# marthinwurer/gcmiipy

Hardware: AMD Instinct MI355X
Metric: cell-updates/s (C-grid Matsuno step) (higher is better)
Workload: dtype f64; 1 GPU; 2-D shallow water + theta + viscosity + van-Leer tracer, 4096x2048 fp64 (BASELINE configs[2]); variant=fused, decomposition=1 latitude band(s)

## Files before the change

gcmiipy_amd/_lib.py:

```python
import ctypes as C
import os

_HERE = os.path.dirname(os.path.abspath(__file__))
LIB_PATH = os.environ.get("GCMCORE_LIB", os.path.join(_HERE, "lib", "libgcmcore.so"))

ABI_VERSION = 1

SW2D, SW2D_TEMP, PE2D, PE25D = 1, 2, 3, 4
P, U, V, T, Q = 0, 1, 2, 3, 4
TRACER_NONE, TRACER_UPWIND, TRACER_VANLEER = 0, 1, 2
VARIANT_AUTO, VARIANT_STAGED, VARIANT_FUSED = 0, 1, 2
F64, F32 = 0, 1
MAX_TRACERS = 16
TRACER_STATS_WORDS = 6
CLIM_WORDS3, CLIM_WORDS2 = 10, 2
PLEV_MAX, PLEV_WORDS, PLEV_PLAN_WORDS = 64, 13, 6
PLEV_MAP_WORDS, PLEV_MAP_WORDS2, PLEV_MAP_PLAN_WORDS = 13, 2, 5
SPEC_WORDS = 6
SPEC_PLAN_WORDS = 6
HDIFF_U, HDIFF_V, HDIFF_T, HDIFF_Q = 1, 2, 4, 8
HDIFF_PLAN_WORDS = 7
SW2D_PLAN_WORDS = 9
PHASE_HELD_SUAREZ, PHASE_MOIST, PHASE_CLIMATE, PHASE_TRACER_FORCING = range(4)
PHASE_PLAN_WORDS = 5
# ... 89 lines not shown
    "gcm_build_info": (C.c_char_p, []),
    "gcm_exner_table": (C.c_int, [_dp]),
    "gcm_filter_plan": (C.c_int, [C.c_int, C.POINTER(C.c_uint), C.c_int]),
    "gcm_create": (C.c_int, [C.POINTER(Config), C.POINTER(_H)]),
    "gcm_destroy": (C.c_int, [_H]),
    "gcm_last_error": (C.c_char_p, [_H]),
    "gcm_set_state": (C.c_int, [_H] + [C.c_void_p] * 5),
    "gcm_get_state": (C.c_int, [_H] + [C.c_void_p] * 5),
    "gcm_members": (C.c_int, [_H]),
    "gcm_set_member": (C.c_int, [_H, C.c_int] + [C.c_void_p] * 5),
    "gcm_get_member": (C.c_int, [_H, C.c_int] + [C.c_void_p] * 5),
    "gcm_diag_members": (C.c_int, [_H, C.c_int, _dp, C.c_int]),
    "gcm_step": (C.c_int, [_H, C.c_int, C.c_double]),
    "gcm_sw2d_plan": (C.c_int, [_H, C.c_int, C.POINTER(C.c_int), C.c_int]),
    "gcm_sw2d_fused_depth": (C.c_int, [_H]),
    "gcm_pe25d_phase_geometry": (C.c_int, [C.c_int] * 7 + [C.POINTER(C.c_int), C.c_int]),
    "gcm_pe25d_phase_plan": (C.c_int, [_H, C.c_int, C.c_int, C.c_int, C.POINTER(C.c_int), C.c_int]),
    "gcm_pe25d_stage_geometry": (C.c_int, [C.c_int] * 5 + [C.POINTER(C.c_uint), C.c_int, C.POINTER(C.c_int), C.c_int]),
    "gcm_pe25d_stage_plan": (C.c_int, [_H, C.POINTER(C.c_int), C.c_int]),
    "gcm_half_step": (C.c_int, [_H, C.c_int, C.c_double]),
    "gcm_end_step": (C.c_int, [_H, C.c_double]),
    "gcm_end_step_diffuse": (C.c_int, [_H, C.c_double]),
    "gcm_end_step_begin": (C.c_int, [_H, C.c_double]),
    "gcm_end_step_finish": (C.c_int, [_H, C.c_double]),
    "gcm_get_star": (C.c_int, [_H] + [C.c_void_p] * 5),
    "gcm_set_star": (C.c_int, [_H] + [C.c_void_p] * 5),
    "gcm_diag": (C.c_int, [_H, C.c_int, _dp]),
    "gcm_energy": (C.c_int, [_H, _dp, C.c_int, _dp]),
    "gcm_stats": (C.c_int, [_H, _dp, C.c_int, _dp]),
    "gcm_flux_limiter": (C.c_int, [C.c_int, C.c_int, C.c_void_p, C.c_void_p, C.c_double, C.c_double, C.c_void_p]),
# ... 168 lines not shown
```

gcmiipy_amd/core.py:

```python
import collections
import ctypes as C

import numpy as np

from . import _lib
from ._lib import lib


class GcmError(RuntimeError):
    pass


def _check(rc, h=None):
    if rc == _lib.OK:
        return
    msg = lib.gcm_last_error(h).decode() if (h or rc) else ""
    if rc == _lib.ERR_ARG:
        raise ValueError(msg or "gcmcore: bad argument")
    raise GcmError("gcmcore error %d: %s" % (rc, msg))


def _count(n, h):
    if n < 0:
        _check(n, h)
# ... 855 lines not shown
    def band_tracer_rows(self):
        return _count(lib.gcm_band_tracer_rows(self._h), self._h)

    @property
    def tracer_count(self):
        return _count(lib.gcm_tracer_count(self._h), self._h)

    def step(self, nsteps, dt):
        _check(lib.gcm_step(self._h, int(nsteps), float(dt)), self._h)

    def sw2d_fused_depth(self):
        d = lib.gcm_sw2d_fused_depth(self._h)
        _check(min(d, 0), self._h)
        return d

    def sw2d_plan(self, nsteps):
        out = (C.c_int * _lib.SW2D_PLAN_WORDS)()
        _check(lib.gcm_sw2d_plan(self._h, int(nsteps), out, _lib.SW2D_PLAN_WORDS), self._h)
        return dict(variant={_lib.VARIANT_FUSED: "fused", _lib.VARIANT_STAGED: "staged"}[out[0]],
                    rows_per_band=out[1], cols=out[2], strip=out[3], strip2=out[4], two_step_launches=out[5],
                    single_step_launches=out[6], preload=bool(out[7]), stream=bool(out[8]))

    def phase_plan(self, phase, rows=None, accumulate=True):
        out = (C.c_int * _lib.PHASE_PLAN_WORDS)()
        _check(lib.gcm_pe25d_phase_plan(self._h, phase_id(phase), -1 if rows is None else int(rows), int(bool(accumulate)),
                                        out, _lib.PHASE_PLAN_WORDS), self._h)
        return _phase_dict(phase_id(phase), out)

    def stage_plan(self):
        out = (C.c_int * _lib.STAGE_PLAN_WORDS)()
# ... 509 lines not shown
```

gcmiipy_amd/csrc/gcm_handle.h:

```cpp
#pragma once
#include "../../include/gcmcore.h"

#include <hip/hip_runtime.h>

#include <algorithm>
#include <cstdio>
#include <string>
#include <vector>

#include "pe25d_kernels.h"
#include "sw2d_kernels.h"

struct GcmBandExchange {
    gcm_exchange xch{};
    bool set = false, primed = false;
    bool inflight = false;
    bool overlap = false;
    hipEvent_t ev_pack = nullptr, ev_comm = nullptr;
    bool join_pending = false;
    bool on_comm = false;
};

struct GcmTiming {
    bool on = false;
// ... 28 lines not shown
    int since_exchange = 0;
    bool ghosts_current = false;
    bool star_valid = false;
    bool launch_refused = false;
    hipStream_t comm = nullptr;
    double *snap[GCM_NFIELDS] = {};
    int snap_since_exchange = 0;
    int variant = GCM_VARIANT_FUSED;
    int rows_per_band = 32;
    int M = 1;
    long mstride = 0;
    bool f32 = false;
    int esz = 8;
    int cols = 1;
    int depth_pin = 0;
    double *staging = nullptr;
    int staging_members = 0;

    double *diag_dev = nullptr;
    static constexpr int kDiagBlocks = 512;

    GcmTiming time;
    gcm::Pe25d *pe = nullptr;
    GcmBandExchange band;
    GcmPhases phases;
};

#define HIPCHK(h, call)                                                                    \
    do {                                                                                   \
        hipError_t e_ = (call);                                                            \
// ... 63 lines not shown
```

gcmiipy_amd/csrc/gcmcore.hip:

```cpp
#include <cmath>
#include <cstdlib>
#include <cstring>

#include "gcm_handle.h"

using namespace gcm;

std::string &gcm_create_error() {
    thread_local std::string e;
    return e;
}

static int alloc_field(gcm_handle *h, double **p) {
    static const long skew_unit = getenv("GCM_ALLOC_SKEW") ? atol(getenv("GCM_ALLOC_SKEW")) : 256;
    const size_t n = all_members_elems(h);
    const size_t skew = (size_t)(skew_unit > 0 ? skew_unit : 0) * (h->allocs.size() % 16) / h->esz;
    void *d = nullptr;
    HIPCHK(h, hipMalloc(&d, (n + skew) * h->esz));
    HIPCHK(h, hipMemsetAsync(d, 0, (n + skew) * h->esz, h->stream));
    h->allocs.push_back(d);
    *p = at(h, (double *)d, (long)(skew + (size_t)h->G * h->W));
    return GCM_OK;
}

// ... 119 lines not shown
                if ((rc = alloc_field(h, &h->cur[f]))) return bail(rc, "");
                if ((rc = alloc_field(h, &h->nxt[f]))) return bail(rc, "");
                if (f != GCM_Q && (rc = alloc_field(h, &h->star[f]))) return bail(rc, "");
            }
            if (temp) {
                if ((rc = alloc_field(h, &h->geo))) return bail(rc, "");
                if ((rc = alloc_field(h, &h->irho))) return bail(rc, "");
                if ((rc = alloc_field(h, &h->sst))) return bail(rc, "");
            }
            if (h->has[GCM_Q] && (rc = alloc_field(h, &h->qtmp))) return bail(rc, "");
            if (temp && !upload_exner_table(h)) return bail(GCM_ERR_HIP, "gcm_create: exner table upload failed");
            const int tr = h->has[GCM_Q] ? cfg->tracer : 0;
            if (h->f32) h->cols = sw2d_fused_cols<float>(h->W, h->H, temp, tr, h->wrap, h->M);
            if (const char *e = getenv("GCM_SW2D_DEPTH"))
                if (temp && !h->f32 && (e[0] == '1' || e[0] == '3') && !e[1]) h->depth_pin = e[0] - '0';
            h->rows_per_band = h->f32 ? sw2d_fused_rows_per_band<float>(h->W, h->H, temp, tr, h->wrap, h->M, h->cols)
                                      : sw2d_fused_rows_per_band<double>(h->W, h->H, temp, tr, h->wrap, h->M, 1, h->depth_pin);
            break;
        }
        case GCM_PE2D: {
            if (!(cfg->dx > 0)) return bail(GCM_ERR_ARG, "gcm_create: dx must be > 0");
            if (cfg->nranks != 1)
                return bail(GCM_ERR_UNSUPPORTED, "gcm_create: GCM_PE2D has no latitude-band mode");
            h->variant = GCM_VARIANT_STAGED;
            for (int f = 0; f < GCM_NFIELDS; ++f) {
                h->has[f] = true;
                if ((rc = alloc_field(h, &h->cur[f]))) return bail(rc, "");
                if ((rc = alloc_field(h, &h->nxt[f]))) return bail(rc, "");
                if ((rc = alloc_field(h, &h->star[f]))) return bail(rc, "");
            }
            if (!upload_exner_table(h)) return bail(GCM_ERR_HIP, "gcm_create: exner table upload failed");
            break;
// ... 139 lines not shown

static void run_derive(const gcm_handle *h, const Sw2dArgs &a, hipStream_t s) {
    if (h->f32) launch_sw2d_derive(narrow_args(a), s);
    else launch_sw2d_derive(a, s);
}
static void run_stage(const gcm_handle *h, const Sw2dArgs &a, bool temp, hipStream_t s) {
    if (h->f32) launch_sw2d_stage(narrow_args(a), temp, s);
    else launch_sw2d_stage(a, temp, s);
}
static void run_tracer_axis(const gcm_handle *h, const Sw2dArgs &a, int axis, bool limit, const double *q_in,
                            double *q_out, hipStream_t s) {
    if (h->f32) launch_tracer_axis(narrow_args(a), axis, limit, (const float *)q_in, (float *)q_out, s);
    else launch_tracer_axis(a, axis, limit, q_in, q_out, s);
}
static bool run_fused(const gcm_handle *h, const Sw2dArgs &a, bool temp, int tracer, hipStream_t s) {
    return h->f32 ? launch_sw2d_fused(narrow_args(a), temp, tracer, s, h->cols) : launch_sw2d_fused(a, temp, tracer, s, 1, h->depth_pin);
}
static bool run_fused2(const gcm_handle *h, const Sw2dArgs &a, hipStream_t s) {
    return h->f32 ? launch_sw2d_fused2(narrow_args(a), s) : launch_sw2d_fused2(a, s);
}

int launch_status(gcm_handle *h) {
    const hipError_t e = hipGetLastError();
    if (h->launch_refused) {
        h->launch_refused = false;
        return fail(h, GCM_ERR_HIP, std::string("sw2d fused kernel: launch refused") +
                                        (e != hipSuccess ? std::string(": ") + hipGetErrorString(e) : std::string()));
    }
    HIPCHK(h, e);
    return GCM_OK;
}
// ... 143 lines not shown
    out[5] = pairs;
    out[6] = nsteps - 2 * pairs;
    out[7] = f.preload;
    out[8] = f.stream;
    return GCM_OK;
}

int gcm_sw2d_fused_depth(gcm_handle *h) {
    if (!h || h->pe) return GCM_ERR_ARG;
    if (h->variant != GCM_VARIANT_FUSED) return 0;
    const int e = step_extra_rows(h);
    return sw2d_fused_form(h->cfg.model == GCM_SW2D_TEMP, h->has[GCM_Q] ? h->cfg.tracer : 0, h->rows_per_band, h->W,
                           h->H + 2 * e, h->M, h->esz, h->depth_pin).depth;
}

int gcm_step_interior(gcm_handle *h, double dt, void *stream) {
    if (!h) return GCM_ERR_ARG;
    if (h->pe) return pe25d_step_part(h->pe, 0, dt, (hipStream_t)stream, &h->err);
    if (h->wrap) return fail(h, GCM_ERR_STATE, "step_interior: handle is not a latitude band");
    if (h->G != kGhost) return fail(h, GCM_ERR_STATE, "step_interior: halo_steps > 1 steps through gcm_step");
    step_rows(h, dt, kGhost, h->H - kGhost, (hipStream_t)stream);
    return launch_status(h);
}

int gcm_step_boundary(gcm_handle *h, double dt, void *stream) {
    if (!h) return GCM_ERR_ARG;
    if (h->pe) return pe25d_step_part(h->pe, 1, dt, (hipStream_t)stream, &h->err);
    if (h->wrap) return fail(h, GCM_ERR_STATE, "step_boundary: handle is not a latitude band");
    hipStream_t s = (hipStream_t)stream;
    if (h->H <= 2 * kGhost) {
// ... 210 lines not shown
```

gcmiipy_amd/csrc/sw2d_impl.h:

```cpp
#pragma once
#include <hip/hip_runtime.h>

#include <cstdlib>
#include <type_traits>

#include "gcm_math.h"
#include "sw2d_kernels.h"

namespace gcm {

__device__ __forceinline__ long row_off(int j, int H, int W, bool wrap) {
    if (wrap) {
        j %= H;
        if (j < 0) j += H;
    }
    return (long)j * W;
}

template <typename T>
__device__ __forceinline__ Sw2dArgsT<T> member_args(const Sw2dArgsT<T> &a0, int m) {
    Sw2dArgsT<T> a = a0;
    const long o = (long)m * a0.mstride;
    auto mv = [o](auto *p) { return p ? p + o : p; };
    a.bu = mv(a.bu); a.bv = mv(a.bv); a.bp = mv(a.bp); a.bt = mv(a.bt); a.bq = mv(a.bq);
// ... 192 lines not shown
};

constexpr unsigned kNoStore = 0x80000000u;
__device__ __forceinline__ void store_row_lanes(double *row, int W, unsigned lane_off, double x) {
    typedef unsigned int u32x2 __attribute__((ext_vector_type(2)));
    const __amdgpu_buffer_rsrc_t rs = __builtin_amdgcn_make_buffer_rsrc(row, 0, W * 8, 0x00020000);
    __builtin_amdgcn_raw_buffer_store_b64(__builtin_bit_cast(u32x2, x), rs, (int)lane_off, 0, 0);
}

__device__ __forceinline__ double own_copy(double x) {
    double y;
    asm volatile("v_mov_b64 %0, %1" : "=v"(y) : "v"(x) : "memory");
    return y;
}

template <typename T, bool TEMP, int TRACER, bool WRAPJ, bool STREAM = false, int CPL = 1>
struct FusedCtx {
    using Real = std::conditional_t<CPL == 2, f32x2, T>;
    using V = Real;
    const Sw2dArgsT<T> &a;
    const double *tab;
    int ci, col, ja, jb;
    bool store_lane;
    V f0_prev;

    __device__ __forceinline__ Raw<V> load(int j) const {
        const long o = row_off(j, a.H, a.W, WRAPJ) + ci;
        Raw<V> r;
        if constexpr (CPL == 2) {
            auto ld = [o](const T *p) {
                const f32x2 *q = (const f32x2 *)(p + o);
                return STREAM ? __builtin_nontemporal_load(q) : *q;
            };
            r.u = ld(a.bu);
            r.v = ld(a.bv);
            r.p = ld(a.bp);
            r.t = TEMP ? ld(a.bt) : V(0.0f);
            r.q = TRACER ? ld(a.bq) : V(0.0f);
        } else if (STREAM) {
            r.u = __builtin_nontemporal_load(&a.bu[o]);
            r.v = __builtin_nontemporal_load(&a.bv[o]);
            r.p = __builtin_nontemporal_load(&a.bp[o]);
            r.t = TEMP ? __builtin_nontemporal_load(&a.bt[o]) : T(0.0);
            r.q = TRACER ? __builtin_nontemporal_load(&a.bq[o]) : T(0.0);
        } else {
            r.u = a.bu[o];
            r.v = a.bv[o];
            r.p = a.bp[o];
            r.t = TEMP ? a.bt[o] : T(0.0);
            r.q = TRACER ? a.bq[o] : T(0.0);
        }
        return r;
    }

// ... 77 lines not shown
};

template <int N, int PRE, class Ctx, typename T = typename Ctx::Real>
__device__ __forceinline__ void preloaded_iters(Ctx &c, const Raw<T> (&pre)[PRE + 4], Row<T> &A, Row<T> &B, Row<T> &C,
                                                Row<T> &X, Row<T> &Y, Row<T> &Z, Raw<T> &nxt, T &qmm, T &qm, T &q0,
                                                T &qp) {
    if constexpr (N < PRE + 2) {
        const int r = c.ja - 1 + N;
        if (r > c.jb) return;
        c.template iter<false>(r, A, B, C, X, Y, Z, nxt, qmm, qm, q0, qp);
        if constexpr (N < PRE) nxt = pre[N + 4];
        preloaded_iters<N + 1, PRE>(c, pre, B, C, A, Y, Z, X, nxt, qmm, qm, q0, qp);
    }
}

template <typename T, bool TEMP, int TRACER, bool WRAPJ, int PRE = 0, bool STREAM = false, int CPL = 1, int DEPTH = 1>
__global__ __launch_bounds__(64, DEPTH == 3 ? 2 : (CPL == 2 && TRACER != 0) ? 3 : 1) void sw2d_fused_kernel(Sw2dArgsT<T> a0) {
    using Ctx = FusedCtx<T, TEMP, TRACER, WRAPJ, STREAM, CPL>;
    using V = typename Ctx::Real;
    constexpr int kCols = sw2d_fused_strip_cols(CPL);
    const int W = a0.W;
    const int lane = threadIdx.x;
    const int strips = (W + kCols - 1) / kCols;
    const int per_xcd = gridDim.x / 8;
    int tile = (blockIdx.x % 8) * per_xcd + blockIdx.x / 8;
    int member = 0;
    if (a0.members > 1) {
        const int per_member = strips * ((a0.j1 - a0.j0 + a0.rows_per_band - 1) / a0.rows_per_band);
        member = tile / per_member;
        if (member >= a0.members) return;
        tile -= member * per_member;
    }
    const int band = tile / strips;
    const int i0 = (tile - band * strips) * kCols;
    const Sw2dArgsT<T> a = member_args(a0, member);
    __shared__ double tab[kExnerTabDoubles];
    if (TEMP) {
        for (int k = 0; k < kExnerTabDoubles / 64; ++k) tab[lane + 64 * k] = a.exner_tab[lane + 64 * k];
        __syncthreads();
    }
    Ctx c{a, tab};
    c.ja = a.j0 + band * a.rows_per_band;
    c.jb = min(c.ja + a.rows_per_band, a.j1);
    if (c.ja >= c.jb) return;
    c.col = i0 - 2 * CPL + CPL * lane;
    c.ci = c.col % W;
    if (c.ci < 0) c.ci += W;
    c.store_lane = lane >= 2 && lane < 62 && c.col < W;
    c.f0_prev = V(0.0);
    const int ja = c.ja, jb = c.jb;

    Row<V> A, B, C, X, Y, Z;
    if constexpr (PRE > 0) {
        Raw<V> pre[PRE + 4];
#pragma unroll
        for (int n = 0; n < PRE + 4; ++n) pre[n] = c.load(min(ja - 2 + n, jb + 1));
        make_row<TEMP>(A, pre[0].u, pre[0].v, pre[0].p, pre[0].t, tab);
        make_row<TEMP>(B, pre[1].u, pre[1].v, pre[1].p, pre[1].t, tab);
        make_row<TEMP>(C, pre[2].u, pre[2].v, pre[2].p, pre[2].t, tab);
        V qmm = V(0.0), qm = pre[0].q, q0 = pre[1].q, qp = pre[2].q;
        Raw<V> nxt = pre[3];
        X = Y = Z = A;
        preloaded_iters<0, PRE>(c, pre, A, B, C, X, Y, Z, nxt, qmm, qm, q0, qp);
        return;
    }
    if constexpr (DEPTH == 3) {
        static_assert(PRE == 0 && CPL == 1, "the deep march is the rolling form with one column per lane");
        const Raw<V> w0 = c.load(ja - 2), w1 = c.load(ja - 1), w2 = c.load(ja);
        Raw<V> n0 = c.load(ja + 1), n1 = c.load(ja + 2), n2 = c.load(min(ja + 3, jb + 1));
        make_row<TEMP>(A, w0.u, w0.v, w0.p, w0.t, tab);
        make_row<TEMP>(B, w1.u, w1.v, w1.p, w1.t, tab);
        make_row<TEMP>(C, w2.u, w2.v, w2.p, w2.t, tab);
        V qmm = V(0.0), qm = w0.q, q0 = w1.q, qp = w2.q;
        X = Y = Z = A;
        c.template iter<true, 5, 0, true>(ja - 1, A, B, C, X, Y, Z, n0, qmm, qm, q0, qp);
        c.template iter<true, 5, 1, true>(ja, B, C, A, Y, Z, X, n1, qmm, qm, q0, qp);
        int r = ja + 1;
        for (; r + 2 <= jb; r += 3) {
            c.template iter<true, 5, 2, true>(r, C, A, B, Z, X, Y, n2, qmm, qm, q0, qp);
            c.template iter<true, 5, 2, true>(r + 1, A, B, C, X, Y, Z, n0, qmm, qm, q0, qp);
            c.template iter<true, 5, 2, true>(r + 2, B, C, A, Y, Z, X, n1, qmm, qm, q0, qp);
        }
        if (r <= jb) {
            c.template iter<false, 3, 2, true>(r, C, A, B, Z, X, Y, n2, qmm, qm, q0, qp);
            if (r + 1 <= jb) c.template iter<false, 3, 2, true>(r + 1, A, B, C, X, Y, Z, n0, qmm, qm, q0, qp);
        }
        return;
    }
    Raw<V> x = c.load(ja - 2);
    make_row<TEMP>(A, x.u, x.v, x.p, x.t, tab);
    V qmm = V(0.0), qm = x.q;
    x = c.load(ja - 1);
    make_row<TEMP>(B, x.u, x.v, x.p, x.t, tab);
    V q0 = x.q;
    x = c.load(ja);
    make_row<TEMP>(C, x.u, x.v, x.p, x.t, tab);
    V qp = x.q;
    Raw<V> nxt = c.load(ja + 1);
    X = Y = Z = A;

    for (int r = ja - 1; r <= jb; r += 3) {
// ... 115 lines not shown
template <typename T>
bool launch_sw2d_fused2(const Sw2dArgsT<T> &a, hipStream_t s) {
    if (!sw2d_fused2_serves(a.wrap_j, a.j0, a.j1, a.H, a.rows_per_band)) return false;
    const int strips = (a.W + kStrip2Cols - 1) / kStrip2Cols;
    const int bands = (a.H + a.rows_per_band - 1) / a.rows_per_band;
    dim3 g((unsigned)(((long)strips * bands * a.members + 7) / 8 * 8));
    Sw2dArgsT<T> arg = a;
    void *params[] = {&arg};
    const bool ens = a.members > 1;
    const void *fn = a.rows_per_band == 2 ? (ens ? (const void *)sw2d_fused2_kernel<T, 2, true> : (const void *)sw2d_fused2_kernel<T, 2, false>)
                   : a.rows_per_band == 3 ? (ens ? (const void *)sw2d_fused2_kernel<T, 3, true> : (const void *)sw2d_fused2_kernel<T, 3, false>)
                                          : (ens ? (const void *)sw2d_fused2_kernel<T, 4, true> : (const void *)sw2d_fused2_kernel<T, 4, false>);
    return hipLaunchKernel(fn, g, dim3(64), params, 0, s) == hipSuccess;
}

template <typename T, bool TEMP, int TRACER, int CPL = 1>
static const void *fused_fn(bool wrap, bool stream, int depth = 1) {
    if constexpr (std::is_same_v<T, double> && TEMP && CPL == 1) {
        if (depth == 3) {
            if (stream)
                return wrap ? (const void *)sw2d_fused_kernel<T, TEMP, TRACER, true, 0, true, CPL, 3>
                            : (const void *)sw2d_fused_kernel<T, TEMP, TRACER, false, 0, true, CPL, 3>;
            return wrap ? (const void *)sw2d_fused_kernel<T, TEMP, TRACER, true, 0, false, CPL, 3>
                        : (const void *)sw2d_fused_kernel<T, TEMP, TRACER, false, 0, false, CPL, 3>;
        }
    }
    if (stream)
        return wrap ? (const void *)sw2d_fused_kernel<T, TEMP, TRACER, true, 0, true, CPL>
                    : (const void *)sw2d_fused_kernel<T, TEMP, TRACER, false, 0, true, CPL>;
    return wrap ? (const void *)sw2d_fused_kernel<T, TEMP, TRACER, true, 0, false, CPL>
                : (const void *)sw2d_fused_kernel<T, TEMP, TRACER, false, 0, false, CPL>;
}

template <typename T, int CPL>
static const void *fused_kernel_ptr_c(bool temp, int tracer, bool wrap, bool preload, bool stream, int depth) {
    if (!temp) {
        if (preload)
            return wrap ? (const void *)sw2d_fused_kernel<T, false, 0, true, kPreloadRows, false, CPL>
                        : (const void *)sw2d_fused_kernel<T, false, 0, false, kPreloadRows, false, CPL>;
        return fused_fn<T, false, 0, CPL>(wrap, stream);
    }
    if (tracer == 0) return fused_fn<T, true, 0, CPL>(wrap, stream, depth);
    if (tracer == 1) return fused_fn<T, true, 1, CPL>(wrap, stream, depth);
    return fused_fn<T, true, 2, CPL>(wrap, stream, depth);
}

template <typename T>
static const void *fused_kernel_ptr(bool temp, int tracer, bool wrap, bool preload = false, bool stream = false,
                                    int cols = 1, int depth = 1) {
    if constexpr (std::is_same_v<T, float>)
        if (cols == 2) return fused_kernel_ptr_c<T, 2>(temp, tracer, wrap, preload, stream, 1);
    return fused_kernel_ptr_c<T, 1>(temp, tracer, wrap, preload, stream, depth);
}

constexpr int kDeepMaxRows = 96;
template <typename T>
int sw2d_fused_rows_per_band(int W, int H, bool temp, int tracer, bool wrap, int members, int cols, int depth_pin) {
    if (const char *e = getenv("GCM_FUSED_ROWS")) {
        int v = atoi(e);
        if (v > 0) return v;
    }
    const long M = members < 1 ? 1 : members;
    const Sw2dFusedForm form = sw2d_fused_form(temp, tracer, kPreloadRows + 1, W, H, M, (long)sizeof(T), depth_pin);
    const bool deep = form.depth == 3;
    int waves_per_cu = deep ? 8 : 12, cus = 256, dev = 0;
    hipDeviceProp_t prop;
    if (hipGetDevice(&dev) == hipSuccess && hipGetDeviceProperties(&prop, dev) == hipSuccess)
        cus = prop.multiProcessorCount;
    int nb = 0;
    if (hipOccupancyMaxActiveBlocksPerMultiprocessor(&nb, fused_kernel_ptr<T>(temp, tracer, wrap, false, deep && form.stream, cols, form.depth),
                                                     64, 0) == hipSuccess && nb > 0)
        waves_per_cu = nb;
    const long slots = (long)waves_per_cu * cus;
    const long strips = (W + sw2d_fused_strip_cols(cols) - 1) / sw2d_fused_strip_cols(cols);
    auto waves = [&](int rpb) { return M * strips * ((H + rpb - 1) / rpb); };
    if (deep && waves(8) >= slots) {
        for (long rounds = 1;; ++rounds) {
            long bands = rounds * slots / (strips * M);
            if (bands < 1) bands = 1;
            const long rpb = (H + bands - 1) / bands;
            if (rpb <= kDeepMaxRows || bands >= H) return (int)(rpb < 8 ? 8 : rpb);
        }
    }
    if (waves(8) < slots) {
        long rpb = M * H * strips / (5L * cus);
        if (!temp && M > 1 && rpb > kPreloadRows) rpb = kPreloadRows;
        return (int)(rpb < 2 ? 2 : rpb > 8 ? 8 : rpb);
// ... 10 lines not shown
    if (!std::is_same_v<T, float> || W % 2) return 1;
    if (const char *e = getenv("GCM_SW2D_F32_COLS")) return e[0] == '1' ? 1 : 2;
    int waves_per_cu = 12, cus = 256, dev = 0, nb = 0;
    hipDeviceProp_t prop;
    if (hipGetDevice(&dev) == hipSuccess && hipGetDeviceProperties(&prop, dev) == hipSuccess)
        cus = prop.multiProcessorCount;
    if (hipOccupancyMaxActiveBlocksPerMultiprocessor(&nb, fused_kernel_ptr<T>(temp, tracer, wrap), 64, 0) == hipSuccess &&
        nb > 0)
        waves_per_cu = nb;
    const long strips = (W + kStripCols - 1) / kStripCols;
    const long waves8 = (long)(members < 1 ? 1 : members) * strips * ((H + 7) / 8);
    return waves8 < (long)waves_per_cu * cus ? 1 : 2;
}

template <typename T>
bool launch_sw2d_fused(const Sw2dArgsT<T> &a, bool temp, int tracer, hipStream_t s, int cols, int depth_pin) {
    if (a.j1 <= a.j0) return true;
    const int strips = (a.W + sw2d_fused_strip_cols(cols) - 1) / sw2d_fused_strip_cols(cols);
    const int bands = (a.j1 - a.j0 + a.rows_per_band - 1) / a.rows_per_band;
    dim3 g((unsigned)(((long)strips * bands * a.members + 7) / 8 * 8));
    Sw2dArgsT<T> arg = a;
    void *params[] = {&arg};
    const Sw2dFusedForm f = sw2d_fused_form(temp, tracer, a.rows_per_band, a.W, a.j1 - a.j0, a.members, (long)sizeof(T), depth_pin);
    return hipLaunchKernel(fused_kernel_ptr<T>(temp, tracer, a.wrap_j != 0, f.preload, f.stream, cols, f.depth), g, dim3(64), params, 0, s) == hipSuccess;
}

template <typename T>
__global__ void copy_rows_kernel(T *dst, const T *src, long n) {
    long i = (long)blockIdx.x * blockDim.x + threadIdx.x;
    const long stride = (long)gridDim.x * blockDim.x;
    for (; i < n; i += stride) dst[i] = src[i];
}

template <typename T>
void launch_copy_rows(T *dst, const T *src, int W, int nrows, hipStream_t s) {
    const long n = (long)W * nrows;
    if (n <= 0) return;
    int blocks = (int)((n + 255) / 256);
    if (blocks > 1024) blocks = 1024;
    hipLaunchKernelGGL(copy_rows_kernel<T>, dim3(blocks), dim3(256), 0, s, dst, src, n);
}

#define GCM_SW2D_INSTANTIATE(T)                                                                                   \
    template void launch_sw2d_stage<T>(const Sw2dArgsT<T> &, bool, hipStream_t);                                 \
    template void launch_sw2d_derive<T>(const Sw2dArgsT<T> &, hipStream_t);                                      \
    template void launch_tracer_axis<T>(const Sw2dArgsT<T> &, int, bool, const T *, T *, hipStream_t);           \
    template bool launch_sw2d_fused<T>(const Sw2dArgsT<T> &, bool, int, hipStream_t, int, int);                  \
    template int sw2d_fused_rows_per_band<T>(int, int, bool, int, bool, int, int, int);                         \
    template int sw2d_fused_cols<T>(int, int, bool, int, bool, int);                                            \
    template bool launch_sw2d_fused2<T>(const Sw2dArgsT<T> &, hipStream_t);                                      \
    template void launch_copy_rows<T>(T *, const T *, int, int, hipStream_t);

}
```

gcmiipy_amd/csrc/sw2d_kernels.h:

```cpp
#pragma once
#include <hip/hip_runtime.h>

namespace gcm {

constexpr int kExnerTabDoubles = 256;
constexpr int kGhost = 2;
constexpr int kStripCols = 60;

constexpr int kStrip2Cols = 56;
constexpr int kPreloadRows = 4;

constexpr int sw2d_fused_strip_cols(int cols) { return cols * kStripCols; }
inline bool sw2d_fused2_serves(int wrap_j, int j0, int j1, int H, int rows_per_band) {
    return wrap_j && j0 == 0 && j1 == H && rows_per_band >= 2 && rows_per_band <= 4;
}
struct Sw2dFusedForm {
    bool preload, stream;
    int depth;
};
inline Sw2dFusedForm sw2d_fused_form(bool temp, int tracer, int rows_per_band, long W, long rows, long members,
                                     long esz, int pin = 0) {
    const int nfields = 3 + (temp ? 1 : 0) + (tracer ? 1 : 0);
    const bool preload = !temp && rows_per_band <= kPreloadRows;
    const bool stream = !preload && W * rows * members * esz * nfields > (256L << 20);
    const bool deep = temp && esz == 8 && !preload && W < (1L << 27) && (pin ? pin == 3 : stream && members == 1);
    return {preload, stream, deep ? 3 : 1};
}

template <typename T>
struct Sw2dArgsT {
    const T *bu, *bv, *bp, *bt, *bq;
    const T *su, *sv, *sp, *st;
    const T *sgeo, *sirho, *sst;
    T *ou, *ov, *op, *ot, *oq;
    T *dgeo, *dirho, *dst;
    const double *exner_tab;
    int W, H;
    int wrap_j;
    int j0, j1;
    int rows_per_band;
    int members;
// ... 16 lines not shown
    f.exner_tab = a.exner_tab;
    f.W = a.W; f.H = a.H; f.wrap_j = a.wrap_j; f.j0 = a.j0; f.j1 = a.j1;
    f.rows_per_band = a.rows_per_band; f.members = a.members; f.mstride = a.mstride;
    f.dt = (float)a.dt; f.dx = (float)a.dx; f.inv_dx = (float)a.inv_dx; f.dx2 = (float)a.dx2;
    f.inv_dx2 = (float)a.inv_dx2; f.h_dx = (float)a.h_dx; f.dtdx = (float)a.dtdx; f.g_dx = (float)a.g_dx;
    f.mu_dx2 = (float)a.mu_dx2; f.inv_dx2_ = (float)a.inv_dx2_;
    return f;
}

template <typename T> void launch_sw2d_stage(const Sw2dArgsT<T> &a, bool temp, hipStream_t s);
template <typename T> void launch_sw2d_derive(const Sw2dArgsT<T> &a, hipStream_t s);
template <typename T>
void launch_tracer_axis(const Sw2dArgsT<T> &a, int axis, bool limit, const T *q_in, T *q_out, hipStream_t s);
template <typename T>
bool launch_sw2d_fused(const Sw2dArgsT<T> &a, bool temp, int tracer, hipStream_t s, int cols = 1,
                       int depth_pin = 0);
template <typename T>
int sw2d_fused_rows_per_band(int W, int H, bool temp, int tracer, bool wrap, int members = 1, int cols = 1,
                             int depth_pin = 0);
template <typename T> int sw2d_fused_cols(int W, int H, bool temp, int tracer, bool wrap, int members);
template <typename T> bool launch_sw2d_fused2(const Sw2dArgsT<T> &a, hipStream_t s);
void launch_narrow(float *dst, long pitch, const double *src, long n, int M, hipStream_t s);
void launch_widen(double *dst, const float *src, long pitch, long n, int M, hipStream_t s);

void launch_pe2d_stage(const double *const base[5], const double *const stage[5], double *const out[5],
                       const double *exner_tab, int W, int H, double dt, double dx, hipStream_t s);

void build_exner_table(double *tab);

template <typename T> void launch_copy_rows(T *dst, const T *src, int W, int nrows, hipStream_t s);

struct SegCopy {
    double *dst[44];
    const double *src[44];
// ... 7 lines not shown
```

include/gcmcore.h:

```cpp
#ifndef GCMCORE_H
#define GCMCORE_H

#include <stddef.h>
#include <stdint.h>

#ifdef __cplusplus
extern "C" {
#endif

#define GCM_ABI_VERSION 1

typedef struct gcm_handle gcm_handle;

typedef enum {
    GCM_OK = 0,
    GCM_ERR_ARG = -1,
    GCM_ERR_HIP = -2,
    GCM_ERR_NODEVICE = -3,
    GCM_ERR_STATE = -4,
    GCM_ERR_UNSUPPORTED = -5
} gcm_status;

typedef enum {
    GCM_SW2D = 1,
// ... 63 lines not shown
int gcm_set_state(gcm_handle *h, const double *p, const double *u, const double *v,
                  const double *t, const double *q);
int gcm_get_state(gcm_handle *h, double *p, double *u, double *v, double *t, double *q);

int gcm_members(const gcm_handle *h);
int gcm_set_member(gcm_handle *h, int m, const double *p, const double *u, const double *v,
                   const double *t, const double *q);
int gcm_get_member(gcm_handle *h, int m, double *p, double *u, double *v, double *t, double *q);

int gcm_step(gcm_handle *h, int nsteps, double dt);

#define GCM_SW2D_PLAN_WORDS 9
int gcm_sw2d_plan(gcm_handle *h, int nsteps, int *out, int nout);

int gcm_sw2d_fused_depth(gcm_handle *h);

typedef enum { GCM_PHASE_HELD_SUAREZ = 0, GCM_PHASE_MOIST = 1, GCM_PHASE_CLIMATE = 2, GCM_PHASE_TRACER_FORCING = 3 } gcm_pe25d_phase;
#define GCM_PHASE_PLAN_WORDS 5
int gcm_pe25d_phase_geometry(int phase, int W, int rows, int L, int cus, int elem_bytes, int accumulate, int *out, int nout);
int gcm_pe25d_phase_plan(gcm_handle *h, int phase, int rows, int accumulate, int *out, int nout);

enum {
    GCM_STAGE_K1_LOOP = 0, GCM_STAGE_K1_MAXR = 1, GCM_STAGE_K1_MASK = 2, GCM_STAGE_K1_NIN = 3, GCM_STAGE_K1_NW = 4,
    GCM_STAGE_K1_PASSES = 5, GCM_STAGE_K1_WGS_PER_ROW = 6, GCM_STAGE_K1_PAIRS_PER_WG = 7, GCM_STAGE_K1_PAIRS_LAST_WG = 8,
    GCM_STAGE_K1_PIT_RIDES = 9,
    GCM_STAGE_K4_ROWS = 10, GCM_STAGE_K4_GROUPS = 11, GCM_STAGE_K4_ROWS_LAST_GROUP = 12, GCM_STAGE_K4_COL_TILES = 13,
    GCM_STAGE_K4_COLS_LAST_TILE = 14, GCM_STAGE_K4_NSEG = 15, GCM_STAGE_K4_ODDTOP = 16, GCM_STAGE_K4_GRID = 17,
    GCM_STAGE_BAND = 18, GCM_STAGE_K1_SPLIT = 19, GCM_STAGE_K1_OWN_WGS_PER_ROW = 20, GCM_STAGE_K1_OWN_PAIRS_PER_WG = 21,
    GCM_STAGE_K1_OWN_PAIRS_LAST_WG = 22,
    GCM_STAGE_K4_EDGE_GROUPS = 23, GCM_STAGE_K4_EDGE_ROWS_LAST_GROUP = 24, GCM_STAGE_K4_EDGE_ODDTOP = 25,
// ... 292 lines not shown
```

Measured before the change: 66.06 billion cell-updates/s.

## Group deep-march waves into 4-wave workgroups with lockstep barriers

For the depth-3 rolling march used on large streaming fp64 grids, adjacent column strips of the same band are now packed into one multi-wave workgroup (four waves by default) instead of one wave per workgroup. By default the waves also synchronise with a workgroup barrier every three rows so they march in lockstep. The intent is that neighbouring strips share halo cache lines in L2 at the same time, and that the exner table load is spread across more lanes. The cost is barrier stalls and coarser scheduling granularity. Environment variables can pin the load hint, group size and lockstep mode, and new query APIs report the chosen settings.

Result: slower. 64.97 billion cell-updates/s (-1.7%).

```diff
diff --git a/gcmiipy_amd/_lib.py b/gcmiipy_amd/_lib.py
--- a/gcmiipy_amd/_lib.py
+++ b/gcmiipy_amd/_lib.py
@@ -127,6 +127,9 @@
     "gcm_step": (C.c_int, [_H, C.c_int, C.c_double]),
     "gcm_sw2d_plan": (C.c_int, [_H, C.c_int, C.POINTER(C.c_int), C.c_int]),
     "gcm_sw2d_fused_depth": (C.c_int, [_H]),
+    "gcm_sw2d_fused_group": (C.c_int, [_H]),
+    "gcm_sw2d_fused_lockstep": (C.c_int, [_H]),
+    "gcm_sw2d_load_hint": (C.c_int, [_H]),
     "gcm_pe25d_phase_geometry": (C.c_int, [C.c_int] * 7 + [C.POINTER(C.c_int), C.c_int]),
     "gcm_pe25d_phase_plan": (C.c_int, [_H, C.c_int, C.c_int, C.c_int, C.POINTER(C.c_int), C.c_int]),
     "gcm_pe25d_stage_geometry": (C.c_int, [C.c_int] * 5 + [C.POINTER(C.c_uint), C.c_int, C.POINTER(C.c_int), C.c_int]),
diff --git a/gcmiipy_amd/core.py b/gcmiipy_amd/core.py
--- a/gcmiipy_amd/core.py
+++ b/gcmiipy_amd/core.py
@@ -893,6 +893,21 @@
         _check(min(d, 0), self._h)
         return d
 
+    def sw2d_fused_group(self):
+        n = lib.gcm_sw2d_fused_group(self._h)
+        _check(min(n, 0), self._h)
+        return n
+
+    def sw2d_fused_lockstep(self):
+        n = lib.gcm_sw2d_fused_lockstep(self._h)
+        _check(min(n, 0), self._h)
+        return bool(n)
+
+    def sw2d_load_hint(self):
+        n = lib.gcm_sw2d_load_hint(self._h)
+        _check(min(n, 0), self._h)
+        return "nt" if n else "plain"
+
     def sw2d_plan(self, nsteps):
         out = (C.c_int * _lib.SW2D_PLAN_WORDS)()
         _check(lib.gcm_sw2d_plan(self._h, int(nsteps), out, _lib.SW2D_PLAN_WORDS), self._h)
diff --git a/gcmiipy_amd/csrc/gcm_handle.h b/gcmiipy_amd/csrc/gcm_handle.h
--- a/gcmiipy_amd/csrc/gcm_handle.h
+++ b/gcmiipy_amd/csrc/gcm_handle.h
@@ -66,6 +66,7 @@
     int esz = 8;
     int cols = 1;
     int depth_pin = 0;
+    gcm::Sw2dDeepPins deep_pins;
     double *staging = nullptr;
     int staging_members = 0;
 
diff --git a/gcmiipy_amd/csrc/gcmcore.hip b/gcmiipy_amd/csrc/gcmcore.hip
--- a/gcmiipy_amd/csrc/gcmcore.hip
+++ b/gcmiipy_amd/csrc/gcmcore.hip
@@ -157,8 +157,16 @@
             if (h->f32) h->cols = sw2d_fused_cols<float>(h->W, h->H, temp, tr, h->wrap, h->M);
             if (const char *e = getenv("GCM_SW2D_DEPTH"))
                 if (temp && !h->f32 && (e[0] == '1' || e[0] == '3') && !e[1]) h->depth_pin = e[0] - '0';
+            if (temp && !h->f32) {
+                if (const char *e = getenv("GCM_SW2D_LOAD_HINT"))
+                    h->deep_pins.hint = !strcmp(e, "nt") ? 1 : !strcmp(e, "plain") ? 2 : 0;
+                if (const char *e = getenv("GCM_SW2D_GROUP"))
+                    if ((e[0] == '1' || e[0] == '2' || e[0] == '4') && !e[1]) h->deep_pins.group = e[0] - '0';
+                if (const char *e = getenv("GCM_SW2D_LOCKSTEP"))
+                    if ((e[0] == '0' || e[0] == '1') && !e[1]) h->deep_pins.lockstep = e[0] - '0';
+            }
             h->rows_per_band = h->f32 ? sw2d_fused_rows_per_band<float>(h->W, h->H, temp, tr, h->wrap, h->M, h->cols)
-                                      : sw2d_fused_rows_per_band<double>(h->W, h->H, temp, tr, h->wrap, h->M, 1, h->depth_pin);
+                                      : sw2d_fused_rows_per_band<double>(h->W, h->H, temp, tr, h->wrap, h->M, 1, h->depth_pin, h->deep_pins);
             break;
         }
         case GCM_PE2D: {
@@ -328,7 +336,7 @@
     else launch_tracer_axis(a, axis, limit, q_in, q_out, s);
 }
 static bool run_fused(const gcm_handle *h, const Sw2dArgs &a, bool temp, int tracer, hipStream_t s) {
-    return h->f32 ? launch_sw2d_fused(narrow_args(a), temp, tracer, s, h->cols) : launch_sw2d_fused(a, temp, tracer, s, 1, h->depth_pin);
+    return h->f32 ? launch_sw2d_fused(narrow_args(a), temp, tracer, s, h->cols) : launch_sw2d_fused(a, temp, tracer, s, 1, h->depth_pin, h->deep_pins);
 }
 static bool run_fused2(const gcm_handle *h, const Sw2dArgs &a, hipStream_t s) {
     return h->f32 ? launch_sw2d_fused2(narrow_args(a), s) : launch_sw2d_fused2(a, s);
@@ -502,6 +510,28 @@
                            h->H + 2 * e, h->M, h->esz, h->depth_pin).depth;
 }
 
+static Sw2dDeepMarch deep_march_of(gcm_handle *h) {
+    const int e = step_extra_rows(h);
+    const Sw2dFusedForm f = sw2d_fused_form(h->cfg.model == GCM_SW2D_TEMP, h->has[GCM_Q] ? h->cfg.tracer : 0, h->rows_per_band,
+                                            h->W, h->H + 2 * e, h->M, h->esz, h->depth_pin);
+    return sw2d_deep_march(f, h->M, h->deep_pins);
+}
+
+int gcm_sw2d_fused_group(gcm_handle *h) {
+    if (!h || h->pe) return GCM_ERR_ARG;
+    return h->variant == GCM_VARIANT_FUSED ? deep_march_of(h).group : 0;
+}
+
+int gcm_sw2d_fused_lockstep(gcm_handle *h) {
+    if (!h || h->pe) return GCM_ERR_ARG;
+    return h->variant == GCM_VARIANT_FUSED && deep_march_of(h).lockstep;
+}
+
+int gcm_sw2d_load_hint(gcm_handle *h) {
+    if (!h || h->pe) return GCM_ERR_ARG;
+    return h->variant == GCM_VARIANT_FUSED && deep_march_of(h).nt;
+}
+
 int gcm_step_interior(gcm_handle *h, double dt, void *stream) {
     if (!h) return GCM_ERR_ARG;
     if (h->pe) return pe25d_step_part(h->pe, 0, dt, (hipStream_t)stream, &h->err);
diff --git a/gcmiipy_amd/csrc/sw2d_impl.h b/gcmiipy_amd/csrc/sw2d_impl.h
--- a/gcmiipy_amd/csrc/sw2d_impl.h
+++ b/gcmiipy_amd/csrc/sw2d_impl.h
@@ -230,7 +230,7 @@
     return y;
 }
 
-template <typename T, bool TEMP, int TRACER, bool WRAPJ, bool STREAM = false, int CPL = 1>
+template <typename T, bool TEMP, int TRACER, bool WRAPJ, bool NT = false, int CPL = 1>
 struct FusedCtx {
     using Real = std::conditional_t<CPL == 2, f32x2, T>;
     using V = Real;
@@ -246,14 +246,14 @@
         if constexpr (CPL == 2) {
             auto ld = [o](const T *p) {
                 const f32x2 *q = (const f32x2 *)(p + o);
-                return STREAM ? __builtin_nontemporal_load(q) : *q;
+                return NT ? __builtin_nontemporal_load(q) : *q;
             };
             r.u = ld(a.bu);
             r.v = ld(a.bv);
             r.p = ld(a.bp);
             r.t = TEMP ? ld(a.bt) : V(0.0f);
             r.q = TRACER ? ld(a.bq) : V(0.0f);
-        } else if (STREAM) {
+        } else if (NT) {
             r.u = __builtin_nontemporal_load(&a.bu[o]);
             r.v = __builtin_nontemporal_load(&a.bv[o]);
             r.p = __builtin_nontemporal_load(&a.bp[o]);
@@ -361,35 +361,56 @@
     }
 }
 
-template <typename T, bool TEMP, int TRACER, bool WRAPJ, int PRE = 0, bool STREAM = false, int CPL = 1, int DEPTH = 1>
-__global__ __launch_bounds__(64, DEPTH == 3 ? 2 : (CPL == 2 && TRACER != 0) ? 3 : 1) void sw2d_fused_kernel(Sw2dArgsT<T> a0) {
-    using Ctx = FusedCtx<T, TEMP, TRACER, WRAPJ, STREAM, CPL>;
+template <typename T, bool TEMP, int TRACER, bool WRAPJ, int PRE = 0, bool NT = false, int CPL = 1, int DEPTH = 1,
+          int NW = 1, bool LOCK = false>
+__global__ __launch_bounds__(64 * NW, DEPTH == 3 ? 2 : (CPL == 2 && TRACER != 0) ? 3 : 1) void sw2d_fused_kernel(Sw2dArgsT<T> a0) {
+    static_assert(NW == 1 || DEPTH == 3, "only the deep march is grouped");
+    static_assert(!LOCK || NW > 1, "lockstep is between the waves of a group");
+    using Ctx = FusedCtx<T, TEMP, TRACER, WRAPJ, NT, CPL>;
     using V = typename Ctx::Real;
     constexpr int kCols = sw2d_fused_strip_cols(CPL);
     const int W = a0.W;
-    const int lane = threadIdx.x;
+    const int lane = NW == 1 ? threadIdx.x : threadIdx.x % 64;
     const int strips = (W + kCols - 1) / kCols;
     const int per_xcd = gridDim.x / 8;
     int tile = (blockIdx.x % 8) * per_xcd + blockIdx.x / 8;
+    [[maybe_unused]] int owed = 0;
+    if constexpr (NW > 1) {
+        tile *= NW;
+        if constexpr (LOCK) {
+            const int ja0 = a0.j0 + (tile / strips) * a0.rows_per_band;
+            const int jb0 = min(ja0 + a0.rows_per_band, a0.j1);
+            owed = jb0 > ja0 ? (jb0 - ja0 - 1) / 3 : 0;
+        }
+        tile += __builtin_amdgcn_readfirstlane(threadIdx.x / 64);
+    }
     int member = 0;
-    if (a0.members > 1) {
-        const int per_member = strips * ((a0.j1 - a0.j0 + a0.rows_per_band - 1) / a0.rows_per_band);
-        member = tile / per_member;
-        if (member >= a0.members) return;
-        tile -= member * per_member;
+    if constexpr (NW == 1) {
+        if (a0.members > 1) {
+            const int per_member = strips * ((a0.j1 - a0.j0 + a0.rows_per_band - 1) / a0.rows_per_band);
+            member = tile / per_member;
+            if (member >= a0.members) return;
+            tile -= member * per_member;
+        }
     }
     const int band = tile / strips;
     const int i0 = (tile - band * strips) * kCols;
     const Sw2dArgsT<T> a = member_args(a0, member);
     __shared__ double tab[kExnerTabDoubles];
     if (TEMP) {
-        for (int k = 0; k < kExnerTabDoubles / 64; ++k) tab[lane + 64 * k] = a.exner_tab[lane + 64 * k];
+        if constexpr (NW == 1) {
+            for (int k = 0; k < kExnerTabDoubles / 64; ++k) tab[lane + 64 * k] = a.exner_tab[lane + 64 * k];
+        } else {
+            for (int k = 0; k < kExnerTabDoubles / (64 * NW); ++k)
+                tab[threadIdx.x + 64 * NW * k] = a.exner_tab[threadIdx.x + 64 * NW * k];
+        }
         __syncthreads();
     }
     Ctx c{a, tab};
     c.ja = a.j0 + band * a.rows_per_band;
     c.jb = min(c.ja + a.rows_per_band, a.j1);
-    if (c.ja >= c.jb) return;
+    if constexpr (NW == 1)
+        if (c.ja >= c.jb) return;
     c.col = i0 - 2 * CPL + CPL * lane;
     c.ci = c.col % W;
     if (c.ci < 0) c.ci += W;
@@ -413,25 +434,36 @@
     }
     if constexpr (DEPTH == 3) {
         static_assert(PRE == 0 && CPL == 1, "the deep march is the rolling form with one column per lane");
-        const Raw<V> w0 = c.load(ja - 2), w1 = c.load(ja - 1), w2 = c.load(ja);
-        Raw<V> n0 = c.load(ja + 1), n1 = c.load(ja + 2), n2 = c.load(min(ja + 3, jb + 1));
-        make_row<TEMP>(A, w0.u, w0.v, w0.p, w0.t, tab);
-        make_row<TEMP>(B, w1.u, w1.v, w1.p, w1.t, tab);
-        make_row<TEMP>(C, w2.u, w2.v, w2.p, w2.t, tab);
-        V qmm = V(0.0), qm = w0.q, q0 = w1.q, qp = w2.q;
-        X = Y = Z = A;
-        c.template iter<true, 5, 0, true>(ja - 1, A, B, C, X, Y, Z, n0, qmm, qm, q0, qp);
-        c.template iter<true, 5, 1, true>(ja, B, C, A, Y, Z, X, n1, qmm, qm, q0, qp);
-        int r = ja + 1;
-        for (; r + 2 <= jb; r += 3) {
-            c.template iter<true, 5, 2, true>(r, C, A, B, Z, X, Y, n2, qmm, qm, q0, qp);
-            c.template iter<true, 5, 2, true>(r + 1, A, B, C, X, Y, Z, n0, qmm, qm, q0, qp);
-            c.template iter<true, 5, 2, true>(r + 2, B, C, A, Y, Z, X, n1, qmm, qm, q0, qp);
-        }
-        if (r <= jb) {
-            c.template iter<false, 3, 2, true>(r, C, A, B, Z, X, Y, n2, qmm, qm, q0, qp);
-            if (r + 1 <= jb) c.template iter<false, 3, 2, true>(r + 1, A, B, C, X, Y, Z, n0, qmm, qm, q0, qp);
-        }
+        if (NW == 1 || ja < jb) {
+            const Raw<V> w0 = c.load(ja - 2), w1 = c.load(ja - 1), w2 = c.load(ja);
+            Raw<V> n0 = c.load(ja + 1), n1 = c.load(ja + 2), n2 = c.load(min(ja + 3, jb + 1));
+            make_row<TEMP>(A, w0.u, w0.v, w0.p, w0.t, tab);
+            make_row<TEMP>(B, w1.u, w1.v, w1.p, w1.t, tab);
+            make_row<TEMP>(C, w2.u, w2.v, w2.p, w2.t, tab);
+            V qmm = V(0.0), qm = w0.q, q0 = w1.q, qp = w2.q;
+            X = Y = Z = A;
+            c.template iter<true, 5, 0, true>(ja - 1, A, B, C, X, Y, Z, n0, qmm, qm, q0, qp);
+            c.template iter<true, 5, 1, true>(ja, B, C, A, Y, Z, X, n1, qmm, qm, q0, qp);
+            int r = ja + 1;
+            for (; r + 2 <= jb; r += 3) {
+                c.template iter<true, 5, 2, true>(r, C, A, B, Z, X, Y, n2, qmm, qm, q0, qp);
+                c.template iter<true, 5, 2, true>(r + 1, A, B, C, X, Y, Z, n0, qmm, qm, q0, qp);
+                c.template iter<true, 5, 2, true>(r + 2, B, C, A, Y, Z, X, n1, qmm, qm, q0, qp);
+                if constexpr (NW > 1 && !LOCK) asm volatile("" ::: "memory");
+                if constexpr (LOCK) {
+                    if (owed > 0) {
+                        __builtin_amdgcn_s_barrier();
+                        --owed;
+                    }
+                }
+            }
+            if (r <= jb) {
+                c.template iter<false, 3, 2, true>(r, C, A, B, Z, X, Y, n2, qmm, qm, q0, qp);
+                if (r + 1 <= jb) c.template iter<false, 3, 2, true>(r + 1, A, B, C, X, Y, Z, n0, qmm, qm, q0, qp);
+            }
+        }
+        if constexpr (LOCK)
+            for (; owed > 0; --owed) __builtin_amdgcn_s_barrier();
         return;
     }
     Raw<V> x = c.load(ja - 2);
@@ -577,15 +609,24 @@
     return hipLaunchKernel(fn, g, dim3(64), params, 0, s) == hipSuccess;
 }
 
+template <typename T, int TRACER, bool WRAPJ, bool NT>
+static const void *deep_fn(int group, bool lockstep) {
+    if (group == 4)
+        return lockstep ? (const void *)sw2d_fused_kernel<T, true, TRACER, WRAPJ, 0, NT, 1, 3, 4, true>
+                        : (const void *)sw2d_fused_kernel<T, true, TRACER, WRAPJ, 0, NT, 1, 3, 4, false>;
+    if (group == 2)
+        return lockstep ? (const void *)sw2d_fused_kernel<T, true, TRACER, WRAPJ, 0, NT, 1, 3, 2, true>
+                        : (const void *)sw2d_fused_kernel<T, true, TRACER, WRAPJ, 0, NT, 1, 3, 2, false>;
+    return (const void *)sw2d_fused_kernel<T, true, TRACER, WRAPJ, 0, NT, 1, 3>;
+}
+
 template <typename T, bool TEMP, int TRACER, int CPL = 1>
-static const void *fused_fn(bool wrap, bool stream, int depth = 1) {
+static const void *fused_fn(bool wrap, bool stream, int depth = 1, int group = 1, bool lockstep = false) {
     if constexpr (std::is_same_v<T, double> && TEMP && CPL == 1) {
         if (depth == 3) {
             if (stream)
-                return wrap ? (const void *)sw2d_fused_kernel<T, TEMP, TRACER, true, 0, true, CPL, 3>
-                            : (const void *)sw2d_fused_kernel<T, TEMP, TRACER, false, 0, true, CPL, 3>;
-            return wrap ? (const void *)sw2d_fused_kernel<T, TEMP, TRACER, true, 0, false, CPL, 3>
-                        : (const void *)sw2d_fused_kernel<T, TEMP, TRACER, false, 0, false, CPL, 3>;
+                return wrap ? deep_fn<T, TRACER, true, true>(group, lockstep) : deep_fn<T, TRACER, false, true>(group, lockstep);
+            return wrap ? deep_fn<T, TRACER, true, false>(group, lockstep) : deep_fn<T, TRACER, false, false>(group, lockstep);
         }
     }
     if (stream)
@@ -596,29 +637,31 @@
 }
 
 template <typename T, int CPL>
-static const void *fused_kernel_ptr_c(bool temp, int tracer, bool wrap, bool preload, bool stream, int depth) {
+static const void *fused_kernel_ptr_c(bool temp, int tracer, bool wrap, bool preload, bool stream, int depth,
+                                      int group = 1, bool lockstep = false) {
     if (!temp) {
         if (preload)
             return wrap ? (const void *)sw2d_fused_kernel<T, false, 0, true, kPreloadRows, false, CPL>
                         : (const void *)sw2d_fused_kernel<T, false, 0, false, kPreloadRows, false, CPL>;
         return fused_fn<T, false, 0, CPL>(wrap, stream);
     }
-    if (tracer == 0) return fused_fn<T, true, 0, CPL>(wrap, stream, depth);
-    if (tracer == 1) return fused_fn<T, true, 1, CPL>(wrap, stream, depth);
-    return fused_fn<T, true, 2, CPL>(wrap, stream, depth);
+    if (tracer == 0) return fused_fn<T, true, 0, CPL>(wrap, stream, depth, group, lockstep);
+    if (tracer == 1) return fused_fn<T, true, 1, CPL>(wrap, stream, depth, group, lockstep);
+    return fused_fn<T, true, 2, CPL>(wrap, stream, depth, group, lockstep);
 }
 
 template <typename T>
 static const void *fused_kernel_ptr(bool temp, int tracer, bool wrap, bool preload = false, bool stream = false,
-                                    int cols = 1, int depth = 1) {
+                                    int cols = 1, int depth = 1, int group = 1, bool lockstep = false) {
     if constexpr (std::is_same_v<T, float>)
         if (cols == 2) return fused_kernel_ptr_c<T, 2>(temp, tracer, wrap, preload, stream, 1);
-    return fused_kernel_ptr_c<T, 1>(temp, tracer, wrap, preload, stream, depth);
+    return fused_kernel_ptr_c<T, 1>(temp, tracer, wrap, preload, stream, depth, group, lockstep);
 }
 
 constexpr int kDeepMaxRows = 96;
 template <typename T>
-int sw2d_fused_rows_per_band(int W, int H, bool temp, int tracer, bool wrap, int members, int cols, int depth_pin) {
+int sw2d_fused_rows_per_band(int W, int H, bool temp, int tracer, bool wrap, int members, int cols, int depth_pin,
+                             const Sw2dDeepPins &pins) {
     if (const char *e = getenv("GCM_FUSED_ROWS")) {
         int v = atoi(e);
         if (v > 0) return v;
@@ -626,14 +669,15 @@
     const long M = members < 1 ? 1 : members;
     const Sw2dFusedForm form = sw2d_fused_form(temp, tracer, kPreloadRows + 1, W, H, M, (long)sizeof(T), depth_pin);
     const bool deep = form.depth == 3;
+    const Sw2dDeepMarch dm = sw2d_deep_march(form, M, pins);
     int waves_per_cu = deep ? 8 : 12, cus = 256, dev = 0;
     hipDeviceProp_t prop;
     if (hipGetDevice(&dev) == hipSuccess && hipGetDeviceProperties(&prop, dev) == hipSuccess)
         cus = prop.multiProcessorCount;
     int nb = 0;
-    if (hipOccupancyMaxActiveBlocksPerMultiprocessor(&nb, fused_kernel_ptr<T>(temp, tracer, wrap, false, deep && form.stream, cols, form.depth),
-                                                     64, 0) == hipSuccess && nb > 0)
-        waves_per_cu = nb;
+    if (hipOccupancyMaxActiveBlocksPerMultiprocessor(&nb, fused_kernel_ptr<T>(temp, tracer, wrap, false, deep && dm.nt, cols, form.depth, dm.group, dm.lockstep),
+                                                     64 * dm.group, 0) == hipSuccess && nb > 0)
+        waves_per_cu = nb * dm.group;
     const long slots = (long)waves_per_cu * cus;
     const long strips = (W + sw2d_fused_strip_cols(cols) - 1) / sw2d_fused_strip_cols(cols);
     auto waves = [&](int rpb) { return M * strips * ((H + rpb - 1) / rpb); };
@@ -674,15 +718,19 @@
 }
 
 template <typename T>
-bool launch_sw2d_fused(const Sw2dArgsT<T> &a, bool temp, int tracer, hipStream_t s, int cols, int depth_pin) {
+bool launch_sw2d_fused(const Sw2dArgsT<T> &a, bool temp, int tracer, hipStream_t s, int cols, int depth_pin,
+                       const Sw2dDeepPins &pins) {
     if (a.j1 <= a.j0) return true;
     const int strips = (a.W + sw2d_fused_strip_cols(cols) - 1) / sw2d_fused_strip_cols(cols);
     const int bands = (a.j1 - a.j0 + a.rows_per_band - 1) / a.rows_per_band;
-    dim3 g((unsigned)(((long)strips * bands * a.members + 7) / 8 * 8));
     Sw2dArgsT<T> arg = a;
     void *params[] = {&arg};
     const Sw2dFusedForm f = sw2d_fused_form(temp, tracer, a.rows_per_band, a.W, a.j1 - a.j0, a.members, (long)sizeof(T), depth_pin);
-    return hipLaunchKernel(fused_kernel_ptr<T>(temp, tracer, a.wrap_j != 0, f.preload, f.stream, cols, f.depth), g, dim3(64), params, 0, s) == hipSuccess;
+    const Sw2dDeepMarch dm = sw2d_deep_march(f, a.members, pins);
+    const long tiles = (long)strips * bands * a.members;
+    dim3 g((unsigned)(((tiles + dm.group - 1) / dm.group + 7) / 8 * 8));
+    return hipLaunchKernel(fused_kernel_ptr<T>(temp, tracer, a.wrap_j != 0, f.preload, dm.nt, cols, f.depth, dm.group, dm.lockstep), g,
+                           dim3(64 * dm.group), params, 0, s) == hipSuccess;
 }
 
 template <typename T>
@@ -705,8 +753,8 @@
     template void launch_sw2d_stage<T>(const Sw2dArgsT<T> &, bool, hipStream_t);                                 \
     template void launch_sw2d_derive<T>(const Sw2dArgsT<T> &, hipStream_t);                                      \
     template void launch_tracer_axis<T>(const Sw2dArgsT<T> &, int, bool, const T *, T *, hipStream_t);           \
-    template bool launch_sw2d_fused<T>(const Sw2dArgsT<T> &, bool, int, hipStream_t, int, int);                  \
-    template int sw2d_fused_rows_per_band<T>(int, int, bool, int, bool, int, int, int);                         \
+    template bool launch_sw2d_fused<T>(const Sw2dArgsT<T> &, bool, int, hipStream_t, int, int, const Sw2dDeepPins &); \
+    template int sw2d_fused_rows_per_band<T>(int, int, bool, int, bool, int, int, int, const Sw2dDeepPins &);   \
     template int sw2d_fused_cols<T>(int, int, bool, int, bool, int);                                            \
     template bool launch_sw2d_fused2<T>(const Sw2dArgsT<T> &, hipStream_t);                                      \
     template void launch_copy_rows<T>(T *, const T *, int, int, hipStream_t);
diff --git a/gcmiipy_amd/csrc/sw2d_kernels.h b/gcmiipy_amd/csrc/sw2d_kernels.h
--- a/gcmiipy_amd/csrc/sw2d_kernels.h
+++ b/gcmiipy_amd/csrc/sw2d_kernels.h
@@ -25,6 +25,26 @@
     const bool stream = !preload && W * rows * members * esz * nfields > (256L << 20);
     const bool deep = temp && esz == 8 && !preload && W < (1L << 27) && (pin ? pin == 3 : stream && members == 1);
     return {preload, stream, deep ? 3 : 1};
+}
+
+constexpr int kDeepGroupDefault = 4;
+constexpr bool kDeepLockstepDefault = true;
+struct Sw2dDeepPins {
+    int hint = 0;
+    int group = 0;
+    int lockstep = -1;
+};
+struct Sw2dDeepMarch {
+    bool nt;
+    int group;
+    bool lockstep;
+};
+inline Sw2dDeepMarch sw2d_deep_march(const Sw2dFusedForm &f, long members, const Sw2dDeepPins &pins) {
+    if (f.depth != 3) return {f.stream, 1, false};
+    const bool nt = pins.hint ? pins.hint == 1 : f.stream;
+    const int group = members > 1 ? 1 : pins.group ? pins.group : f.stream ? kDeepGroupDefault : 1;
+    const bool lockstep = group > 1 && (pins.lockstep >= 0 ? pins.lockstep != 0 : kDeepLockstepDefault);
+    return {nt, group, lockstep};
 }
 
 template <typename T>
@@ -71,10 +91,10 @@
 void launch_tracer_axis(const Sw2dArgsT<T> &a, int axis, bool limit, const T *q_in, T *q_out, hipStream_t s);
 template <typename T>
 bool launch_sw2d_fused(const Sw2dArgsT<T> &a, bool temp, int tracer, hipStream_t s, int cols = 1,
-                       int depth_pin = 0);
+                       int depth_pin = 0, const Sw2dDeepPins &deep = Sw2dDeepPins());
 template <typename T>
 int sw2d_fused_rows_per_band(int W, int H, bool temp, int tracer, bool wrap, int members = 1, int cols = 1,
-                             int depth_pin = 0);
+                             int depth_pin = 0, const Sw2dDeepPins &deep = Sw2dDeepPins());
 template <typename T> int sw2d_fused_cols(int W, int H, bool temp, int tracer, bool wrap, int members);
 template <typename T> bool launch_sw2d_fused2(const Sw2dArgsT<T> &a, hipStream_t s);
 void launch_narrow(float *dst, long pitch, const double *src, long n, int M, hipStream_t s);
diff --git a/include/gcmcore.h b/include/gcmcore.h
--- a/include/gcmcore.h
+++ b/include/gcmcore.h
@@ -101,6 +101,10 @@
 int gcm_sw2d_plan(gcm_handle *h, int nsteps, int *out, int nout);
 
 int gcm_sw2d_fused_depth(gcm_handle *h);
+
+int gcm_sw2d_fused_group(gcm_handle *h);
+int gcm_sw2d_fused_lockstep(gcm_handle *h);
+int gcm_sw2d_load_hint(gcm_handle *h);
 
 typedef enum { GCM_PHASE_HELD_SUAREZ = 0, GCM_PHASE_MOIST = 1, GCM_PHASE_CLIMATE = 2, GCM_PHASE_TRACER_FORCING = 3 } gcm_pe25d_phase;
 #define GCM_PHASE_PLAN_WORDS 5
```
